# tkkim-robot/safe_control

Measured on AMD Instinct MI355X. Metric: QP solves/sec (batched agents), higher is better.
Workload: dtype f64; 1 GPU; 4096-agent batch DynamicUnicycle2D CBF-QP, 8 obstacles each (BASELINE configs[1]); agents_per_gpu=4096, obstacles=8, storage=f32, arithmetic=f64, launch=hipGraph

## Files before the change

safe_control_amd/csrc/cbf_qp_kernel.hpp:

```cpp
#pragma once
#include <hip/hip_runtime.h>

#include <type_traits>
#include <utility>

#include <cstdlib>

#include "sc_qp2.hpp"
#include "sc_group.hpp"

namespace sc {

#ifndef SC_COOP_MAX_AGENTS
#define SC_COOP_MAX_AGENTS 32768
#endif

static inline long long sc_coop_max_agents() {
    static const long long v = [] { const char* e = getenv("SC_COOP_MAX_AGENTS"); return e ? atoll(e) : (long long)SC_COOP_MAX_AGENTS; }();
    return v;
}
static inline bool sc_two_pass() {
    static const bool v = [] { const char* e = getenv("SC_CBFQP_TWO_PASS"); return !(e && e[0] == '0'); }();
    return v;
}
// ... 189 lines not shown
    const bool has_row = sub < K;
    const TIO* src = obs + (obs_shared ? 0 : (size_t)ag_i * K * 7) + (has_row ? sub * 7 : 0);
#pragma unroll
    for (int f = 0; f < 7; ++f) orow[f] = src[f];
    const V2 ur = reinterpret_cast<const V2*>(u_ref)[ag_i];
    const StateRow<TIO, MODEL> xs = load_state<TIO, MODEL>(X, ag_i);
    int nk = K;
    if (n_obs) nk = n_obs[ag_i];
    nk = nk < 0 ? 0 : (nk > K ? K : nk);
    fetch_arg_now(status_out); fetch_arg_now(h_out);
    fetch_arg_now(k.R); fetch_arg_now(k.g1); fetch_arg_now(k.g2);
    fetch_arg_now(k.lo0); fetch_arg_now(k.hi0); fetch_arg_now(k.lo1); fetch_arg_now(k.hi1); fetch_arg_now(k.hard);
#ifdef SC_EXP_LOADS
    if (active) {
        if (sub == 0) {
            V2 uo; uo.x = ur.x + xs.v[0] + xs.v[1]; uo.y = ur.y + xs.v[2] + xs.v[3];
            reinterpret_cast<V2*>(u_out)[agent] = uo;
            status_out[agent] = nk;
        }
        if (h_out && has_row) h_out[agent * K + sub] = orow[0] + orow[1] + orow[2] + orow[3] + orow[4] + orow[5] + orow[6];
    }
    return;
#endif
    const TC ur0 = TC(ur.x), ur1 = TC(ur.y);
    const Agent<TC> ag = to_agent<TIO, TC, MODEL>(xs);

    TC o[7];
#pragma unroll
    for (int f = 0; f < 7; ++f) o[f] = TC(orow[f]);
    TC h, a0, a1, cc;
#ifndef SC_EXP_NOROW
    const bool ok = cbf_row<TC, MODEL, false>(ag, o, k, a0, a1, cc, h);
#else
    const bool ok = true; a0 = o[0] - ag.x; a1 = o[1] - ag.y; cc = o[2]; h = o[3];
#endif
    const bool used = sub < nk;
    const bool bad_mine = used && !ok;
    a0 = used ? a0 : TC(0); a1 = used ? a1 : TC(0); cc = used ? cc : TC(0);
    if (active && h_out && has_row) h_out[agent * K + sub] = used ? TIO(h) : TIO(0);
    TC poison = TC(0);
    normalise_row(a0, a1, cc, poison);

    QpState<TC> S;
    qp_begin(S, ur0, ur1, k);
#ifndef SC_EXP_NOWALK
#ifndef SC_COOP_OLD_WALK
    if constexpr (G == 8) coop_solve_all8<TC>(S, K, sub, lane, a0, a1, cc, k);
    else if constexpr (G == 16) coop_solve_all16<TC>(S, K, sub, lane, a0, a1, cc, k);
    else
#endif
    coop_walk_violated<TC, G>(S, K, sub, lane, a0, a1, cc, k);
#endif
    qp_finish_box(S, k);
    TC worst = qp_row_margin(num<TC>::inf(), a0, a1, cc, S.u0, S.u1, poison);
    const bool nan_mine = !(poison == poison);
    worst = nan_mine ? -num<TC>::inf() : worst;
    if constexpr (G == 8) worst = min8_raw(worst);
    else if constexpr (G == 16) worst = min16_raw(worst);
    else worst = group_min<TC, G>(worst);
    const unsigned long long bad_mask = __builtin_amdgcn_ballot_w64(bad_mine);
    const bool bad_any = ((bad_mask >> (lane & ~(G - 1))) & (G == 64 ? ~0ull : ((1ull << G) - 1ull))) != 0ull;
    int st = qp_status(S, worst, TC(0), k);
    if (bad_any) st = SC_STATUS_BAD_OBSTACLE;
    TC u0 = S.u0, u1 = S.u1;
    if (st != SC_STATUS_OPTIMAL) { u0 = num<TC>::nan(); u1 = num<TC>::nan(); }
    if (active) {
        if (sub == 0) {
            V2 uo; uo.x = TIO(u0); uo.y = TIO(u1);
            reinterpret_cast<V2*>(u_out)[agent] = uo;
            status_out[agent] = st;
        }
    }
}

typedef double sc_d8 __attribute__((ext_vector_type(8)));
struct Coop8Consts {
    sc_d8 t0;
    sc_d8 t1;
    sc_d8 k0;
    sc_d8 k1;
    unsigned B;
};

__device__ __forceinline__ void normalise_row_as_generic(double& n0, double& n1, double& c, double& poison) {
    const double nn = __builtin_fma(n1, n1, n0 * n0);
    poison += 0.0 * (nn + c);
    double inv = rsqrt_(nn);
    if (__builtin_amdgcn_ballot_w64(!(nn > 0.0)) != 0ull) {
        asm volatile("");
        inv = nn > 0.0 ? inv : 1.0;
    }
    n0 *= inv; n1 *= inv; c *= inv;
}

template <typename T>
__device__ __forceinline__ T* at_byte(T* base, unsigned off) {
    using C = typename std::conditional<std::is_const<T>::value, const char, char>::type;
    return reinterpret_cast<T*>(reinterpret_cast<C*>(base) + off);
}

template <typename TIO, bool FULL, bool HAS_H, bool HARD>
__global__ __launch_bounds__(64) void cbfqp_coop8_du_kernel(const TIO* __restrict__ obs, const TIO* __restrict__ X,
                                                            const TIO* __restrict__ u_ref, TIO* __restrict__ u_out,
                                                            TIO* __restrict__ h_out, int* __restrict__ status_out,
                                                            const Coop8Consts c) {
#ifdef SC_EXP_EMPTY
    return;
#endif
    using TC = double;
    using V2 = typename vec2<TIO>::type;
    const unsigned lane = threadIdx.x;
    const unsigned sub = lane & 7u;
    const unsigned slot = blockIdx.x * 64u + lane;
    const unsigned agent = slot >> 3;
    bool active = true;
    if constexpr (!FULL) active = agent < c.B;
    const unsigned row_i = active ? slot : sub;
    const unsigned ag8 = row_i & ~7u;

    struct { TIO v[7]; } orow;
    __builtin_memcpy(&orow, at_byte(obs, __umul24(row_i, 7u * (unsigned)sizeof(TIO))), sizeof(orow));
    const V2 ur = *reinterpret_cast<const V2*>(at_byte(u_ref, ag8 * (unsigned)(sizeof(V2) / 8)));
    StateRow<TIO, SC_MODEL_DYNAMIC_UNICYCLE2D> xs;
    __builtin_memcpy(&xs, at_byte(X, ag8 * (unsigned)(sizeof(xs) / 8)), sizeof(xs));
    fetch_arg_now(c.t0); fetch_arg_now(c.t1); fetch_arg_now(c.k0); fetch_arg_now(c.k1);

    SinCosTab sc;
    sc.two_over_pi = c.t0[0]; sc.pio2_1 = c.t0[1]; sc.pio2_2 = c.t0[2]; sc.pio2_3 = c.t0[3];
    sc.s[0] = c.t0[4]; sc.s[1] = c.t0[5]; sc.s[2] = c.t0[6]; sc.s[3] = c.t0[7]; sc.s[4] = c.t1[0]; sc.s[5] = c.t1[1];
#pragma unroll
    for (int i = 0; i < 6; ++i) sc.c[i] = c.t1[2 + i];
    CbfConsts<TC> k;
    k.R = c.k0[0]; k.a1 = TC(0); k.a2 = TC(0); k.g1 = c.k0[1]; k.g2 = c.k0[2]; k.inv_dt = c.k0[3]; k.inv_dt2 = c.k0[4];
    k.lo0 = c.k0[5]; k.hi0 = c.k0[6]; k.lo1 = c.k0[7]; k.hi1 = c.k1[0]; k.inv_Lr = TC(0); k.inv_mass = TC(1); k.hard = HARD;
    BoxTol<TC> bt;
    bt.lo0 = c.k1[1]; bt.hi0 = c.k1[2]; bt.lo1 = c.k1[3]; bt.hi1 = c.k1[4];
    SolveLit<TC> lit;
    lit.tol_feas = c.k1[5]; lit.eps_par = c.k1[6]; lit.inf = c.k1[7];

    const TC ur0 = TC(ur.x), ur1 = TC(ur.y);
    Agent<TC> ag;
    ag.x = TC(xs.v[0]); ag.y = TC(xs.v[1]); ag.th = TC(xs.v[2]); ag.v = TC(xs.v[3]);
    sincos_tab_sfma(ag.th, sc, &ag.s, &ag.c);
    ag.f0 = ag.v * ag.c;
    ag.f1 = ag.v * ag.s;

    TC o[7];
#pragma unroll
    for (int f = 0; f < 7; ++f) o[f] = TC(orow.v[f]);
    TC h, a0, a1, cc;
    const bool ok = cbf_row<TC, SC_MODEL_DYNAMIC_UNICYCLE2D, false>(ag, o, k, a0, a1, cc, h);
    const bool bad_mine = !ok;
    if constexpr (HAS_H) {
        if (active) *at_byte(h_out, slot * (unsigned)sizeof(TIO)) = TIO(h);
    }
    TC poison = TC(0);
    normalise_row_as_generic(a0, a1, cc, poison);

    QpState<TC> S;
    qp_begin_raw(S, ur0, ur1, k);
    coop_solve_all8_full<TC>(S, (int)sub, (int)lane, a0, a1, cc, k, bt, lit);
    qp_finish_box_raw(S, k);
    TC worst = qp_row_margin_raw(a0, a1, cc, S.u0, S.u1, poison, lit);
    const bool nan_mine = !(poison == poison);
    worst = nan_mine ? -num<TC>::inf() : worst;
    worst = min8_raw(worst);
    int st = qp_status_lit(S, worst, TC(0), k, lit);
    if (__builtin_amdgcn_ballot_w64(bad_mine) != 0ull) {
        asm volatile("");
        const unsigned long long bad_mask = __builtin_amdgcn_ballot_w64(bad_mine);
        const bool bad_any = ((bad_mask >> (lane & ~7u)) & 0xffull) != 0ull;
        if (bad_any) st = SC_STATUS_BAD_OBSTACLE;
    }
    TC u0 = S.u0, u1 = S.u1;
    if (st != SC_STATUS_OPTIMAL) { u0 = num<TC>::nan(); u1 = num<TC>::nan(); }
    if (active && sub == 0) {
        V2 uo; uo.x = TIO(u0); uo.y = TIO(u1);
        reinterpret_cast<V2*>(u_out)[agent] = uo;
        status_out[agent] = st;
    }
}

#if defined(SC_EXP_GRID) && !defined(SC_EXP_EMPTY)
#error "SC_EXP_GRID needs SC_EXP_EMPTY: a kernel with a body would run past the batch"
#endif
static inline unsigned coop_grid(unsigned nblk) {
#ifdef SC_EXP_GRID
    return SC_EXP_GRID;
#else
    return nblk;
#endif
}

static inline bool sc_cbfqp_generic() {
    static const bool v = [] { const char* e = getenv("SC_CBFQP_GENERIC"); return e && e[0] == '1'; }();
    return v;
}

static inline double sc_quieted(double x) {
    if (x != x) {
        unsigned long long b;
        __builtin_memcpy(&b, &x, sizeof(b));
        b |= 0x0008000000000000ull;
        __builtin_memcpy(&x, &b, sizeof(b));
    }
    return x;
}

template <typename TIO>
static hipError_t launch_coop8_du(const sc_cbfqp_params& p, long long B, const void* X, const void* u_ref, const void* obs,
                                  void* u_out, int* status, void* h_out, hipStream_t stream) {
    const CbfConsts<double> k = make_consts<double>(p);
    const BoxTol<double> bt = box_tol(k);
    const SinCosTab t = make_sincos_tab();
    Coop8Consts c;
    c.t0 = sc_d8{t.two_over_pi, t.pio2_1, t.pio2_2, t.pio2_3, t.s[0], t.s[1], t.s[2], t.s[3]};
    c.t1 = sc_d8{t.s[4], t.s[5], t.c[0], t.c[1], t.c[2], t.c[3], t.c[4], t.c[5]};
    c.k0 = sc_d8{k.R, k.g1, k.g2, k.inv_dt, k.inv_dt2, sc_quieted(k.lo0), sc_quieted(k.hi0), sc_quieted(k.lo1)};
    c.k1 = sc_d8{sc_quieted(k.hi1), bt.lo0, bt.hi0, bt.lo1, bt.hi1, 1e-9, 1e-12, __builtin_huge_val()};
    c.B = (unsigned)B;
    const dim3 grid(coop_grid((unsigned)((B + 7) / 8))), block(64);
#define SC_GO(FULL, HAS_H, HARD)                                                                                             \
    hipLaunchKernelGGL((cbfqp_coop8_du_kernel<TIO, FULL, HAS_H, HARD>), grid, block, 0, stream, (const TIO*)obs, (const TIO*)X, \
                       (const TIO*)u_ref, (TIO*)u_out, (TIO*)h_out, status, c)
#define SC_GO_H(FULL, HAS_H) do { if (k.hard) SC_GO(FULL, HAS_H, true); else SC_GO(FULL, HAS_H, false); } while (0)
    if (B % 8 == 0) { if (h_out) SC_GO_H(true, true); else SC_GO_H(true, false); }
    else { if (h_out) SC_GO_H(false, true); else SC_GO_H(false, false); }
#undef SC_GO_H
#undef SC_GO
    return hipGetLastError();
}

template <typename TIO, typename TC, int G, int MODEL>
static hipError_t launch_coop(const sc_cbfqp_params& p, long long B, int K, const void* X, const void* u_ref,
                              const void* obs, const int* n_obs, void* u_out, int* status, void* h_out,
                              hipStream_t stream) {
    if constexpr (G == 8 && MODEL == SC_MODEL_DYNAMIC_UNICYCLE2D && sizeof(TC) == 8 && SC_COOP_WAVES == 1) {
        if (K == 8 && n_obs == nullptr && p.obs_shared == 0 && B >= 1 && B <= sc_coop_max_agents() &&
            B * 8 * 7 * (long long)sizeof(TIO) <= 0x7fffffffLL && B * 8 <= 0xffffffLL && !sc_cbfqp_generic())
            return launch_coop8_du<TIO>(p, B, X, u_ref, obs, u_out, status, h_out, stream);
    }
    constexpr int APW = 64 / G;
    const unsigned nblk = coop_grid((unsigned)((B + APW * SC_COOP_WAVES - 1) / (APW * SC_COOP_WAVES)));
    const CbfConsts<TC> k = make_consts<TC>(p);
    hipLaunchKernelGGL((cbfqp_coop_kernel<TIO, TC, G, MODEL>), dim3(nblk), dim3(64 * SC_COOP_WAVES), 0, stream,
                       (const TIO*)obs, (const TIO*)X, (const TIO*)u_ref, n_obs, B, K, (int)p.obs_shared,
                       (TIO*)u_out, status, (TIO*)h_out, k);
    return hipGetLastError();
}

template <typename TIO, typename TC, int KMAX, int MODEL>
__global__ __launch_bounds__(64) void cbfqp_kernel(const TIO* __restrict__ obs, const TIO* __restrict__ X,
                                                   const TIO* __restrict__ u_ref, const int* __restrict__ n_obs,
                                                   const long long B, const int K, const int obs_shared,
                                                   TIO* __restrict__ u_out, int* __restrict__ status_out,
                                                   TIO* __restrict__ h_out, const CbfConsts<TC> k) {
    extern __shared__ __attribute__((aligned(16))) unsigned char smem[];
    TIO* lobs = reinterpret_cast<TIO*>(smem);

    const int lane = threadIdx.x;
    const long long first = (long long)blockIdx.x * 64;
    const long long agent = first + lane;
    const int nag = (int)((B - first) < 64 ? (B - first) : 64);
    const bool active = lane < nag;
    const int row_elems = K * 7;

    if (obs_shared) {
        for (int e = lane; e < row_elems; e += 64) lobs[e] = obs[e];
    } else {
        const TIO* src = obs + (size_t)first * row_elems;
        const unsigned bytes = (unsigned)nag * row_elems * sizeof(TIO);
        if ((bytes & 15u) == 0 && ((reinterpret_cast<uintptr_t>(src) & 15u) == 0)) {
            wave_dma16(reinterpret_cast<const unsigned char*>(src), smem, bytes, lane);
        } else {
            const int total = nag * row_elems;
            for (int e = lane; e < total; e += 64) lobs[e] = src[e];
        }
    }

    using V2 = typename vec2<TIO>::type;
    const long long ag_i = active ? agent : 0;
    const V2 ur = reinterpret_cast<const V2*>(u_ref)[ag_i];
    const StateRow<TIO, MODEL> xs = load_state<TIO, MODEL>(X, ag_i);
    int nk = K;
    if (n_obs) nk = n_obs[ag_i];
    nk = !active ? K : (nk < 0 ? 0 : (nk > K ? K : nk));
    const TC ur0 = active ? TC(ur.x) : TC(0), ur1 = active ? TC(ur.y) : TC(0);
    const Agent<TC> ag = to_agent<TIO, TC, MODEL>(xs);

    asm volatile("s_waitcnt vmcnt(0)" ::: "memory");
    __syncthreads();

    const size_t stage_bytes = ((obs_shared ? (size_t)row_elems : (size_t)64 * row_elems) * sizeof(TIO) + 15) & ~(size_t)15;
    TC* rows = reinterpret_cast<TC*>(smem + stage_bytes);
    TIO* hl = reinterpret_cast<TIO*>(rows + (size_t)K * 3 * 64);
    const TIO* mine = lobs + (obs_shared ? 0 : lane * row_elems);
    int period = 32;
    while (((K * (32 / period)) & 31) != 0 && period > 1) period >>= 1;
    const int rot = obs_shared ? 0 : (lane / period) % K;
    bool bad_obs = false;
    TC poison = TC(0);
#pragma nounroll
// ... 152 lines not shown
```

safe_control_amd/csrc/sc_group.hpp:

```cpp
#pragma once
#include <hip/hip_runtime.h>

#include <utility>

#include "sc_qp2.hpp"

namespace sc {

template <int CTRL>
__device__ __forceinline__ float dpp_mov(float v) {
    return __int_as_float(__builtin_amdgcn_update_dpp(0, __float_as_int(v), CTRL, 0xf, 0xf, true));
}
template <int CTRL>
__device__ __forceinline__ double dpp_mov(double v) {
    const int lo = __builtin_amdgcn_update_dpp(0, __double2loint(v), CTRL, 0xf, 0xf, true);
    const int hi = __builtin_amdgcn_update_dpp(0, __double2hiint(v), CTRL, 0xf, 0xf, true);
    return __hiloint2double(hi, lo);
}
template <typename T, int G, int I>
__device__ __forceinline__ T group_bcast(T v, int sub) {
    if constexpr (G == 8) {
        const T q = dpp_mov<(I & 3) * 0x55>(v);
        const T m = dpp_mov<0x141>(q);
        return ((sub >> 2) == (I >> 2)) ? q : m;
// ... 93 lines not shown
__device__ __forceinline__ double keep_or_nan(bool keep, double v) {
    return __hiloint2double(keep ? __double2hiint(v) : 0x7ff80000, __double2loint(v));
}
template <typename T>
__device__ __forceinline__ T min8_raw(T v) {
    v = min_raw(v, dpp_mov<0xB1>(v)); v = min_raw(v, dpp_mov<0x4E>(v)); v = min_raw(v, dpp_mov<0x141>(v));
    return v;
}
template <typename T>
__device__ __forceinline__ T min16_raw(T v) { v = min8_raw(v); return min_raw(v, dpp_mov<0x140>(v)); }
template <int CTRL>
__device__ __forceinline__ int or_dpp(int v) { return v | __builtin_amdgcn_update_dpp(0, v, CTRL, 0xf, 0xf, true); }
template <int G>
__device__ __forceinline__ int group_or_bits(int v) {
    v = or_dpp<0xB1>(v); v = or_dpp<0x4E>(v); v = or_dpp<0x141>(v);
    if constexpr (G == 16) v = or_dpp<0x140>(v);
    return v;
}
template <int G>
__device__ __forceinline__ float group_pick(bool mine, float v) { return __int_as_float(group_or_bits<G>(mine ? __float_as_int(v) : 0)); }
template <int G>
__device__ __forceinline__ double group_pick(bool mine, double v) {
    const int lo = group_or_bits<G>(mine ? __double2loint(v) : 0), hi = group_or_bits<G>(mine ? __double2hiint(v) : 0);
    return __hiloint2double(hi, lo);
}

template <typename T>
__device__ __forceinline__ void clip_row_coop(LineQP<T>& L, bool& dead, T g0, T g1, T gc) {
    const T a = g0 * L.d0 + g1 * L.d1;
    const T r = g0 * L.p0 + (g1 * L.p1 + gc);
    const bool pos = a > num<T>::eps_par();
    const bool neg = !(a >= -num<T>::eps_par());
    const bool par_viol = r < -num<T>::tol_feas() * max_abs_one_raw(gc);
    const T q = r * rcp_(fabs_(a));
    dead |= !pos && !neg && par_viol;
    L.lo = max_neg_raw(L.lo, keep_or_nan(pos, q));
    L.hi = min_raw(L.hi, keep_or_nan(neg, q));
}

template <int G>
__device__ __forceinline__ bool group_first(unsigned long long m, int lane, int sub, bool& has) {
    const unsigned bits = (unsigned)(m >> (lane & ~(G - 1))) & ((1u << G) - 1u);
    has = bits != 0u;
    return sub == __builtin_ctz(bits | (1u << G));
}

template <typename TC, int... Xs>
__device__ __forceinline__ void clip_partners8(LineQP<TC>& L, bool& dead, TC a0, TC a1, TC cc, std::integer_sequence<int, Xs...>) {
    const TC m0 = dpp_mov<0x141>(a0), m1 = dpp_mov<0x141>(a1), mc = dpp_mov<0x141>(cc);
    (clip_row_coop(L, dead, group_xor8<TC, Xs + 1>(a0, m0), group_xor8<TC, Xs + 1>(a1, m1), group_xor8<TC, Xs + 1>(cc, mc)), ...);
}
template <typename TC, int G>
__device__ __forceinline__ void coop_pick_winner(QpState<TC>& S, const LineQP<TC>& L, bool ok, int sub, int lane) {
    const TC inf = num<TC>::inf();
    TC t = fmin_(fmax_(TC(0), L.lo), L.hi);
    const bool inverted = L.lo > L.hi;
    t = inverted ? TC(0.5) * (L.lo + L.hi) : t;
    const bool empty = L.lo > L.hi + num<TC>::tol_feas() * fmax_(TC(1), fmax_(fabs_(L.lo), fabs_(L.hi)));
    const TC v0 = L.p0 + t * L.d0, v1 = L.p1 + t * L.d1;
    const TC e0 = v0 - S.ur0, e1 = v1 - S.ur1;
    TC cost = e0 * e0 + e1 * e1;
    cost = (ok && !empty && (cost == cost)) ? cost : inf;
    TC best;
    if constexpr (G == 8) best = min8_raw(cost); else best = min16_raw(cost);
    bool has;
    const bool mine = group_first<G>(__builtin_amdgcn_ballot_w64((cost == best) && (best < inf)), lane, sub, has);
    const TC s0 = group_pick<G>(mine, v0), s1 = group_pick<G>(mine, v1);
    S.u0 = has ? s0 : S.u0;
    S.u1 = has ? s1 : S.u1;
}
template <typename TC>
__device__ __forceinline__ void coop_solve_all8(QpState<TC>& S, int K, int sub, int lane, TC a0, TC a1, TC cc,
                                                const CbfConsts<TC>& k) {
    const bool testable = (sub < K) && !((a0 == TC(0)) && (a1 == TC(0)));
    LineQP<TC> L;
    const bool viol = qp_row_violated(S, a0, a1, cc, L, k) && testable;
    if (__builtin_amdgcn_ballot_w64(viol) == 0ull) return;
    clip_box(L, k);
    bool dead = false;
    clip_partners8(L, dead, a0, a1, cc, std::make_integer_sequence<int, 7>{});
    coop_pick_winner<TC, 8>(S, L, viol && !dead, sub, lane);
}

template <typename T>
struct BoxTol { T lo0, hi0, lo1, hi1; };
template <typename T>
__host__ __device__ inline BoxTol<T> box_tol(const CbfConsts<T>& k) {
    const T tol = sizeof(T) == 8 ? T(1e-9) : T(1e-5f);
    BoxTol<T> b;
    b.lo0 = k.lo0 - tol; b.hi0 = k.hi0 + tol; b.lo1 = k.lo1 - tol; b.hi1 = k.hi1 + tol;
    return b;
}
template <typename T>
__device__ __forceinline__ void clip_box_tol(LineQP<T>& L, const CbfConsts<T>& k, const BoxTol<T>& bt) {
    const T inf = num<T>::inf();
    {
        const T r = rcp_(L.d0);
        const T t1 = (k.lo0 - L.p0) * r, t2 = (k.hi0 - L.p0) * r;
        const bool flat = L.d0 == T(0);
        const bool inside = (L.p0 >= bt.lo0) && (L.p0 <= bt.hi0);
        const T lo = flat ? (inside ? -inf : inf) : fmin_(t1, t2);
        const T hi = flat ? inf : fmax_(t1, t2);
        L.lo = lo; L.hi = hi;
    }
    {
        const T r = rcp_(L.d1);
        const T t1 = (k.lo1 - L.p1) * r, t2 = (k.hi1 - L.p1) * r;
        const bool flat = L.d1 == T(0);
        const bool inside = (L.p1 >= bt.lo1) && (L.p1 <= bt.hi1);
        const T lo = flat ? (inside ? -inf : inf) : fmin_(t1, t2);
        const T hi = flat ? inf : fmax_(t1, t2);
        L.lo = fmax_(L.lo, lo); L.hi = fmin_(L.hi, hi);
    }
}

__device__ __forceinline__ double max_raw_s(double a, double b) { double r; asm("v_max_f64 %0, %1, %2" : "=v"(r) : "v"(a), "s"(b)); return r; }
__device__ __forceinline__ double min_raw_s(double a, double b) { double r; asm("v_min_f64 %0, %1, %2" : "=v"(r) : "v"(a), "s"(b)); return r; }
__device__ __forceinline__ double max_zero_raw(double a) { double r; asm("v_max_f64 %0, %1, 0" : "=v"(r) : "v"(a)); return r; }
__device__ __forceinline__ double max_one_raw(double a) { double r; asm("v_max_f64 %0, %1, 1.0" : "=v"(r) : "v"(a)); return r; }
__device__ __forceinline__ double max_abs_abs_raw(double a, double b) { double r; asm("v_max_f64 %0, |%1|, |%2|" : "=v"(r) : "v"(a), "v"(b)); return r; }

__device__ __forceinline__ void qp_begin_raw(QpState<double>& S, double ur0, double ur1, const CbfConsts<double>& k) {
    S.ur0 = ur0; S.ur1 = ur1;
    S.u0 = min_raw_s(max_raw_s(ur0, k.lo0), k.hi0);
    S.u1 = min_raw_s(max_raw_s(ur1, k.lo1), k.hi1);
}
__device__ __forceinline__ void qp_finish_box_raw(QpState<double>& S, const CbfConsts<double>& k) {
    S.u0 = min_raw_s(max_raw_s(S.u0, k.lo0), k.hi0);
    S.u1 = min_raw_s(max_raw_s(S.u1, k.lo1), k.hi1);
}
template <typename T>
struct SolveLit { T tol_feas, eps_par, inf; };

__device__ __forceinline__ double qp_row_margin_raw(double a0, double a1, double ci, double u0, double u1, double& poison,
                                                    const SolveLit<double>& lit) {
    const double s = a0 * u0 + (a1 * u1 + ci);
    const double m = s + lit.tol_feas * max_abs_one_raw(ci);
    poison += 0.0 * s;
    return fmin_(lit.inf, m);
}
__device__ __forceinline__ int qp_status_lit(const QpState<double>& S, double worst, double poison, const CbfConsts<double>& k,
                                             const SolveLit<double>& lit) {
    const bool finite = (poison == poison) && (fabs_(S.ur0 + S.ur1) < lit.inf);
    const bool box_ok = (k.lo0 <= k.hi0) && (k.lo1 <= k.hi1);
    return (!(worst >= 0.0) || !finite || !box_ok) ? SC_STATUS_INFEASIBLE : SC_STATUS_OPTIMAL;
}

template <typename T>
__device__ __forceinline__ void clip_box_tol_lazy(LineQP<T>& L, const CbfConsts<T>& k, const BoxTol<T>& bt) {
    const T r0 = rcp_(L.d0), r1 = rcp_(L.d1);
    const T t1 = (k.lo0 - L.p0) * r0, t2 = (k.hi0 - L.p0) * r0;
    const T t3 = (k.lo1 - L.p1) * r1, t4 = (k.hi1 - L.p1) * r1;
    const bool flat = (L.d0 == T(0)) || (L.d1 == T(0));
    L.lo = fmax_(fmin_(t1, t2), fmin_(t3, t4));
    L.hi = fmin_(fmax_(t1, t2), fmax_(t3, t4));
    if (__builtin_amdgcn_ballot_w64(flat) != 0ull) clip_box_tol(L, k, bt);
}

__device__ __forceinline__ double min_abs_abs_raw(double a, double b) { double r; asm("v_min_f64 %0, |%1|, |%2|" : "=v"(r) : "v"(a), "v"(b)); return r; }
__device__ __forceinline__ double min_abs_raw(double a, double b) { double r; asm("v_min_f64 %0, %1, |%2|" : "=v"(r) : "v"(a), "v"(b)); return r; }
__device__ __forceinline__ double clip_row_coop_lazy(LineQP<double>& L, double eps, double g0, double g1, double gc) {
    const double a = g0 * L.d0 + g1 * L.d1;
    const double r = g0 * L.p0 + (g1 * L.p1 + gc);
    const bool pos = a > eps;
    const bool neg = !(a >= -eps);
    const double q = r * rcp_(fabs_(a));
    L.lo = max_neg_raw(L.lo, keep_or_nan(pos, q));
    L.hi = min_raw(L.hi, keep_or_nan(neg, q));
    return a;
}
template <int X>
__device__ __forceinline__ double clip_partner8_lazy(LineQP<double>& L, double eps, double a0, double a1, double cc, double m0, double m1,
                                                     double mc) {
    return clip_row_coop_lazy(L, eps, group_xor8<double, X>(a0, m0), group_xor8<double, X>(a1, m1), group_xor8<double, X>(cc, mc));
}
__device__ __forceinline__ double clip_partners8_lazy(LineQP<double>& L, double eps, double a0, double a1, double cc) {
    const double m0 = dpp_mov<0x141>(a0), m1 = dpp_mov<0x141>(a1), mc = dpp_mov<0x141>(cc);
    const double x1 = clip_partner8_lazy<1>(L, eps, a0, a1, cc, m0, m1, mc);
    const double x2 = clip_partner8_lazy<2>(L, eps, a0, a1, cc, m0, m1, mc);
    double amin = min_abs_abs_raw(x1, x2);
    amin = min_abs_raw(amin, clip_partner8_lazy<3>(L, eps, a0, a1, cc, m0, m1, mc));
    amin = min_abs_raw(amin, clip_partner8_lazy<4>(L, eps, a0, a1, cc, m0, m1, mc));
    amin = min_abs_raw(amin, clip_partner8_lazy<5>(L, eps, a0, a1, cc, m0, m1, mc));
    amin = min_abs_raw(amin, clip_partner8_lazy<6>(L, eps, a0, a1, cc, m0, m1, mc));
    amin = min_abs_raw(amin, clip_partner8_lazy<7>(L, eps, a0, a1, cc, m0, m1, mc));
    return amin;
}
template <typename T>
__device__ __forceinline__ bool row_dead_coop(const LineQP<T>& L, T g0, T g1, T gc) {
    const T a = g0 * L.d0 + g1 * L.d1;
    const T r = g0 * L.p0 + (g1 * L.p1 + gc);
    const bool pos = a > num<T>::eps_par();
    const bool neg = !(a >= -num<T>::eps_par());
    const bool par_viol = r < -num<T>::tol_feas() * max_abs_one_raw(gc);
    return !pos && !neg && par_viol;
}
template <typename TC>
__device__ __forceinline__ bool partners8_dead(const LineQP<TC>& L, TC a0, TC a1, TC cc) {
    bool dead = false;
#pragma nounroll
    for (int x = 1; x < 8; ++x) dead |= row_dead_coop(L, __shfl_xor(a0, x, 8), __shfl_xor(a1, x, 8), __shfl_xor(cc, x, 8));
    return dead;
}

__device__ __forceinline__ void coop_pick_winner8_raw(QpState<double>& S, const LineQP<double>& L, bool ok, int sub, int lane,
                                                      const SolveLit<double>& lit) {
    using TC = double;
    const TC inf = num<TC>::inf();
    TC t = min_raw(max_zero_raw(L.lo), L.hi);
    const bool inverted = L.lo > L.hi;
    t = inverted ? TC(0.5) * (L.lo + L.hi) : t;
    const bool empty = L.lo > L.hi + lit.tol_feas * max_one_raw(max_abs_abs_raw(L.lo, L.hi));
    const TC v0 = L.p0 + t * L.d0, v1 = L.p1 + t * L.d1;
    const TC e0 = v0 - S.ur0, e1 = v1 - S.ur1;
    TC cost = e0 * e0 + e1 * e1;
    cost = (ok && !empty && (cost == cost)) ? cost : inf;
    const TC best = min8_raw(cost);
    bool has;
    const bool mine = group_first<8>(__builtin_amdgcn_ballot_w64((cost == best) && (best < lit.inf)), lane, sub, has);
    const TC s0 = group_pick<8>(mine, v0), s1 = group_pick<8>(mine, v1);
    S.u0 = has ? s0 : S.u0;
    S.u1 = has ? s1 : S.u1;
}

template <typename TC>
__device__ __forceinline__ void coop_solve_all8_full(QpState<TC>& S, int sub, int lane, TC a0, TC a1, TC cc,
                                                     const CbfConsts<TC>& k, const BoxTol<TC>& bt, const SolveLit<TC>& lit) {
    const bool testable = !((a0 == TC(0)) && (a1 == TC(0)));
    LineQP<TC> L;
    const bool viol = qp_row_violated(S, a0, a1, cc, L, k) && testable;
    if (__builtin_amdgcn_ballot_w64(viol) == 0ull) return;
    clip_box_tol_lazy(L, k, bt);
    const TC amin = clip_partners8_lazy(L, lit.eps_par, a0, a1, cc);
    bool dead = false;
    if (__builtin_amdgcn_ballot_w64(amin <= lit.eps_par) != 0ull)
        dead = partners8_dead(L, a0, a1, cc);
    coop_pick_winner8_raw(S, L, viol && !dead, sub, lane, lit);
}

template <typename TC, int... Rs>
__device__ __forceinline__ void clip_partners16(LineQP<TC>& L, bool& dead, TC a0, TC a1, TC cc, std::integer_sequence<int, Rs...>) {
    (clip_row_coop(L, dead, dpp_mov<0x121 + Rs>(a0), dpp_mov<0x121 + Rs>(a1), dpp_mov<0x121 + Rs>(cc)), ...);
}
template <typename TC>
__device__ __forceinline__ void coop_solve_all16(QpState<TC>& S, int K, int sub, int lane, TC a0, TC a1, TC cc,
                                                 const CbfConsts<TC>& k) {
    const bool testable = (sub < K) && !((a0 == TC(0)) && (a1 == TC(0)));
    LineQP<TC> L;
    const bool viol = qp_row_violated(S, a0, a1, cc, L, k) && testable;
    if (__builtin_amdgcn_ballot_w64(viol) == 0ull) return;
    clip_box(L, k);
    bool dead = false;
    clip_partners16(L, dead, a0, a1, cc, std::make_integer_sequence<int, 15>{});
    coop_pick_winner<TC, 16>(S, L, viol && !dead, sub, lane);
}

}
```

safe_control_amd/csrc/sc_math.hpp:

```cpp
#pragma once
#include <hip/hip_runtime.h>
#include <cmath>
#include <cstdint>

namespace sc {

template <typename T> struct num;
template <> struct num<float> {
    static __device__ __forceinline__ float inf() { return __builtin_huge_valf(); }
    static __device__ __forceinline__ float nan() { return __builtin_nanf(""); }
    static __device__ __forceinline__ float eps_par() { return 1e-5f; }
    static __device__ __forceinline__ float tol_feas() { return 1e-5f; }
};
template <> struct num<double> {
    static __device__ __forceinline__ double inf() { return __builtin_huge_val(); }
    static __device__ __forceinline__ double nan() { return __builtin_nan(""); }
    static __device__ __forceinline__ double eps_par() { return 1e-12; }
    static __device__ __forceinline__ double tol_feas() { return 1e-9; }
};

__device__ __forceinline__ void sincos_(float x, float* s, float* c) { sincosf(x, s, c); }
__device__ __forceinline__ void sincos_(double x, double* s, double* c) {
    if (!(fabs(x) < 1.0e5)) { sincos(x, s, c); return; }
    const double k = rint(x * 0.63661977236758138);
    double r = __builtin_fma(-k, 1.5707963267948966, x);
    r = __builtin_fma(-k, 6.123233995736766e-17, r);
    r = __builtin_fma(-k, -1.4973849048591698e-33, r);
    const double z = r * r;
    double ps = __builtin_fma(z, 1.58969099521155010221e-10, -2.50507602534068634195e-08);
    ps = __builtin_fma(z, ps, 2.75573137070700676789e-06);
    ps = __builtin_fma(z, ps, -1.98412698298579493134e-04);
    ps = __builtin_fma(z, ps, 8.33333333332248946124e-03);
    const double ks = __builtin_fma(z * r, __builtin_fma(z, ps, -1.66666666666666324348e-01), r);
    double pc = __builtin_fma(z, -1.13596475577881948265e-11, 2.08757232129817482790e-09);
    pc = __builtin_fma(z, pc, -2.75573143513906633035e-07);
    pc = __builtin_fma(z, pc, 2.48015872894767294178e-05);
    pc = __builtin_fma(z, pc, -1.38888888888741095749e-03);
    pc = __builtin_fma(z, pc, 4.16666666666666019037e-02);
    const double hz = 0.5 * z, w = 1.0 - hz;
    const double kc = w + (((1.0 - w) - hz) + z * (z * pc));
    const int n = (int)k & 3;
    const double sv = (n & 1) ? kc : ks, cv = (n & 1) ? ks : kc;
    *s = (n & 2) ? -sv : sv;
    *c = ((n + 1) & 2) ? -cv : cv;
}
struct SinCosTab {
    double two_over_pi, pio2_1, pio2_2, pio2_3;
    double s[6];
    double c[6];
};
__host__ __device__ inline SinCosTab make_sincos_tab() {
    SinCosTab t;
    t.two_over_pi = 0.63661977236758138;
    t.pio2_1 = 1.5707963267948966; t.pio2_2 = 6.123233995736766e-17; t.pio2_3 = -1.4973849048591698e-33;
    t.s[0] = 1.58969099521155010221e-10; t.s[1] = -2.50507602534068634195e-08; t.s[2] = 2.75573137070700676789e-06;
    t.s[3] = -1.98412698298579493134e-04; t.s[4] = 8.33333333332248946124e-03; t.s[5] = -1.66666666666666324348e-01;
    t.c[0] = -1.13596475577881948265e-11; t.c[1] = 2.08757232129817482790e-09; t.c[2] = -2.75573143513906633035e-07;
    t.c[3] = 2.48015872894767294178e-05; t.c[4] = -1.38888888888741095749e-03; t.c[5] = 4.16666666666666019037e-02;
    return t;
}
__device__ __forceinline__ void sincos_tab(double x, const SinCosTab& t, double* s, double* c) {
    if (!(fabs(x) < 1.0e5)) { sincos(x, s, c); return; }
    const double k = rint(x * t.two_over_pi);
    double r = __builtin_fma(-k, t.pio2_1, x);
    r = __builtin_fma(-k, t.pio2_2, r);
    r = __builtin_fma(-k, t.pio2_3, r);
    const double z = r * r;
    double ps = __builtin_fma(z, t.s[0], t.s[1]);
    ps = __builtin_fma(z, ps, t.s[2]);
    ps = __builtin_fma(z, ps, t.s[3]);
    ps = __builtin_fma(z, ps, t.s[4]);
    const double ks = __builtin_fma(z * r, __builtin_fma(z, ps, t.s[5]), r);
    double pc = __builtin_fma(z, t.c[0], t.c[1]);
    pc = __builtin_fma(z, pc, t.c[2]);
    pc = __builtin_fma(z, pc, t.c[3]);
    pc = __builtin_fma(z, pc, t.c[4]);
    pc = __builtin_fma(z, pc, t.c[5]);
    const double hz = 0.5 * z, w = 1.0 - hz;
    const double kc = w + (((1.0 - w) - hz) + z * (z * pc));
    const int n = (int)k & 3;
    const double sv = (n & 1) ? kc : ks, cv = (n & 1) ? ks : kc;
    *s = (n & 2) ? -sv : sv;
    *c = ((n + 1) & 2) ? -cv : cv;
}
__device__ __forceinline__ double fma_sconst(double a, double b, double c) {
    double d;
    asm("v_fma_f64 %0, %1, %2, %3" : "=v"(d) : "v"(a), "v"(b), "s"(c));
    return d;
}
__device__ __forceinline__ void sincos_tab_sfma(double x, const SinCosTab& t, double* s, double* c) {
    if (!(fabs(x) < 1.0e5)) { sincos(x, s, c); return; }
    const double k = rint(x * t.two_over_pi);
    double r = __builtin_fma(-k, t.pio2_1, x);
    r = __builtin_fma(-k, t.pio2_2, r);
    r = __builtin_fma(-k, t.pio2_3, r);
    const double z = r * r;
    double ps = __builtin_fma(z, t.s[0], t.s[1]);
    ps = fma_sconst(z, ps, t.s[2]);
    ps = fma_sconst(z, ps, t.s[3]);
    ps = fma_sconst(z, ps, t.s[4]);
    const double ks = __builtin_fma(z * r, fma_sconst(z, ps, t.s[5]), r);
    double pc = __builtin_fma(z, t.c[0], t.c[1]);
    pc = fma_sconst(z, pc, t.c[2]);
    pc = fma_sconst(z, pc, t.c[3]);
    pc = fma_sconst(z, pc, t.c[4]);
    pc = fma_sconst(z, pc, t.c[5]);
    const double hz = 0.5 * z, w = 1.0 - hz;
    const double kc = w + (((1.0 - w) - hz) + z * (z * pc));
    const int n = (int)k & 3;
    const double sv = (n & 1) ? kc : ks, cv = (n & 1) ? ks : kc;
    *s = (n & 2) ? -sv : sv;
    *c = ((n + 1) & 2) ? -cv : cv;
}
__device__ __forceinline__ float sqrt_(float x) { return sqrtf(x); }
__device__ __forceinline__ double sqrt_(double x) { return sqrt(x); }
__device__ __forceinline__ float fabs_(float x) { return fabsf(x); }
__device__ __forceinline__ double fabs_(double x) { return fabs(x); }
__device__ __forceinline__ float fmax_(float a, float b) { return fmaxf(a, b); }
__device__ __forceinline__ double fmax_(double a, double b) { return fmax(a, b); }
__device__ __forceinline__ float fmin_(float a, float b) { return fminf(a, b); }
__device__ __forceinline__ double fmin_(double a, double b) { return fmin(a, b); }
__device__ __forceinline__ float pow_(float a, float b) { return powf(a, b); }
__device__ __forceinline__ double pow_(double a, double b) { return pow(a, b); }
__device__ __forceinline__ float rint_(float a) { return rintf(a); }
__device__ __forceinline__ double rint_(double a) { return rint(a); }
__device__ __forceinline__ float atan2_(float a, float b) { return atan2f(a, b); }
__device__ __forceinline__ double atan2_(double a, double b) { return atan2(a, b); }
__device__ __forceinline__ float floor_(float a) { return floorf(a); }
__device__ __forceinline__ double floor_(double a) { return floor(a); }
__device__ __forceinline__ bool finite_(float a) { return __builtin_isfinite(a); }
__device__ __forceinline__ bool finite_(double a) { return __builtin_isfinite(a); }

template <typename T>
__device__ __forceinline__ T powi_chain(T x, int n) {
    T r = T(1), b = x;
    while (n) {
        if (n & 1) r *= b;
        b *= b;
        n >>= 1;
    }
    return r;
}

__device__ __forceinline__ float fmod_(float a, float b) { return fmodf(a, b); }
__device__ __forceinline__ double fmod_(double a, double b) { return fmod(a, b); }

template <typename T>
__device__ __forceinline__ T pymod(T x, T m) {
    T r = fmod_(x, m);
    if (r < T(0)) r += m;
    return r;
}

template <typename T>
__device__ __forceinline__ T angle_normalize(T x) {
    const T pi = T(3.14159265358979323846);
    return pymod(x + pi, T(2) * pi) - pi;
}

}
```

Measured before the change: 1.682 billion solves/s.

## Split coop8 kernel into fast path with wave-level fallback to generic solver

```diff
diff --git a/safe_control_amd/csrc/cbf_qp_kernel.hpp b/safe_control_amd/csrc/cbf_qp_kernel.hpp
--- a/safe_control_amd/csrc/cbf_qp_kernel.hpp
+++ b/safe_control_amd/csrc/cbf_qp_kernel.hpp
@@ -295,21 +295,74 @@
     unsigned B;
 };
 
-__device__ __forceinline__ void normalise_row_as_generic(double& n0, double& n1, double& c, double& poison) {
+template <bool HARD>
+__device__ __forceinline__ void circle_row_du_as_generic(const Agent<double>& a, const double* o, const CbfConsts<double>& k,
+                                                         double neg_beta, double& n0, double& n1, double& c, double& h) {
+    const double ex = a.x - o[0], ey = a.y - o[1];
+    const double dmin = o[2] + k.R;
+    h = __builtin_fma(dmin, dmin * neg_beta, __builtin_fma(ex, ex, ey * ey));
+    const double hdot = 2.0 * __builtin_fma(ex, a.f0, ey * a.f1);
+    const double dhd0 = 2.0 * a.f0, dhd1 = 2.0 * a.f1;
+    n1 = 2.0 * __builtin_fma(ey, a.f0, -(ex * a.f1));
+    n0 = 2.0 * __builtin_fma(ex, a.c, ey * a.s);
+    const double Lf = __builtin_fma(dhd0, a.f0, dhd1 * a.f1);
+    if constexpr (HARD) c = __builtin_fma(h, k.inv_dt2, (2.0 * hdot) * k.inv_dt) + Lf;
+    else c = __builtin_fma(k.g2, h, __builtin_fma(k.g1, hdot, Lf));
+}
+
+__device__ __forceinline__ bool normalise_row_fast(double& n0, double& n1, double& c, double& poison) {
     const double nn = __builtin_fma(n1, n1, n0 * n0);
     poison += 0.0 * (nn + c);
-    double inv = rsqrt_(nn);
-    if (__builtin_amdgcn_ballot_w64(!(nn > 0.0)) != 0ull) {
-        asm volatile("");
-        inv = nn > 0.0 ? inv : 1.0;
-    }
+    const double inv = rsqrt_(nn);
     n0 *= inv; n1 *= inv; c *= inv;
+    return !(nn > 0.0);
 }
 
 template <typename T>
 __device__ __forceinline__ T* at_byte(T* base, unsigned off) {
     using C = typename std::conditional<std::is_const<T>::value, const char, char>::type;
     return reinterpret_cast<T*>(reinterpret_cast<C*>(base) + off);
+}
+
+template <typename TIO, bool HAS_H>
+__device__ __forceinline__ void coop8_generic_body(const TIO* orow, typename vec2<TIO>::type ur,
+                                                   const StateRow<TIO, SC_MODEL_DYNAMIC_UNICYCLE2D>& xs, bool active,
+                                                   unsigned slot, int sub, int lane, const CbfConsts<double>& k,
+                                                   TIO* __restrict__ h_out, typename vec2<TIO>::type& uo, int& st) {
+    using TC = double;
+    constexpr int MODEL = SC_MODEL_DYNAMIC_UNICYCLE2D;
+    int K = 8, nk = 8;
+    asm volatile("" : "+s"(K), "+s"(nk));
+    const TC ur0 = TC(ur.x), ur1 = TC(ur.y);
+    const Agent<TC> ag = to_agent<TIO, TC, MODEL>(xs);
+    TC o[7];
+#pragma unroll
+    for (int f = 0; f < 7; ++f) o[f] = TC(orow[f]);
+    TC h, a0, a1, cc;
+    const bool ok = cbf_row<TC, MODEL, false>(ag, o, k, a0, a1, cc, h);
+    const bool used = sub < nk;
+    const bool bad_mine = used && !ok;
+    a0 = used ? a0 : TC(0); a1 = used ? a1 : TC(0); cc = used ? cc : TC(0);
+    if constexpr (HAS_H) {
+        if (active && sub < K) *at_byte(h_out, slot * (unsigned)sizeof(TIO)) = used ? TIO(h) : TIO(0);
+    }
+    TC poison = TC(0);
+    normalise_row(a0, a1, cc, poison);
+    QpState<TC> S;
+    qp_begin(S, ur0, ur1, k);
+    coop_solve_all8<TC>(S, K, sub, lane, a0, a1, cc, k);
+    qp_finish_box(S, k);
+    TC worst = qp_row_margin(num<TC>::inf(), a0, a1, cc, S.u0, S.u1, poison);
+    const bool nan_mine = !(poison == poison);
+    worst = nan_mine ? -num<TC>::inf() : worst;
+    worst = min8_raw(worst);
+    const unsigned long long bad_mask = __builtin_amdgcn_ballot_w64(bad_mine);
+    const bool bad_any = ((bad_mask >> (lane & ~7)) & 0xffull) != 0ull;
+    st = qp_status(S, worst, TC(0), k);
+    if (bad_any) st = SC_STATUS_BAD_OBSTACLE;
+    TC u0 = S.u0, u1 = S.u1;
+    if (st != SC_STATUS_OPTIMAL) { u0 = num<TC>::nan(); u1 = num<TC>::nan(); }
+    uo.x = TIO(u0); uo.y = TIO(u1);
 }
 
 template <typename TIO, bool FULL, bool HAS_H, bool HARD>
@@ -338,61 +391,66 @@
     __builtin_memcpy(&xs, at_byte(X, ag8 * (unsigned)(sizeof(xs) / 8)), sizeof(xs));
     fetch_arg_now(c.t0); fetch_arg_now(c.t1); fetch_arg_now(c.k0); fetch_arg_now(c.k1);
 
+    CbfConsts<TC> k;
+    k.R = c.k0[0]; k.a1 = TC(0); k.a2 = TC(0); k.g1 = c.k0[1]; k.g2 = c.k0[2]; k.inv_dt = c.k0[3]; k.inv_dt2 = c.k0[4];
+    k.lo0 = c.k0[5]; k.hi0 = c.k0[6]; k.lo1 = c.k0[7]; k.hi1 = c.k1[0]; k.inv_Lr = TC(0); k.inv_mass = TC(1); k.hard = HARD;
+    SolveLit<TC> lit;
+    lit.th_max = c.k1[1]; lit.neg_beta = c.k1[2]; lit.tol_feas = c.k1[5]; lit.eps_par = c.k1[6]; lit.inf = c.k1[7];
+
+    const TC th = TC(xs.v[2]);
+    const bool early = (orow.v[6] != TIO(0)) || !(fabs(th) < lit.th_max);
+    const auto store_u_status = [&](V2 uo, int st) {
+        if (active && sub == 0) {
+            reinterpret_cast<V2*>(u_out)[agent] = uo;
+            status_out[agent] = st;
+        }
+    };
+    if (__builtin_expect(__builtin_amdgcn_ballot_w64(early) != 0ull, 0)) {
+        V2 uo; int st;
+        coop8_generic_body<TIO, HAS_H>(orow.v, ur, xs, active, slot, (int)sub, (int)lane, k, h_out, uo, st);
+        store_u_status(uo, st);
+        return;
+    }
     SinCosTab sc;
     sc.two_over_pi = c.t0[0]; sc.pio2_1 = c.t0[1]; sc.pio2_2 = c.t0[2]; sc.pio2_3 = c.t0[3];
     sc.s[0] = c.t0[4]; sc.s[1] = c.t0[5]; sc.s[2] = c.t0[6]; sc.s[3] = c.t0[7]; sc.s[4] = c.t1[0]; sc.s[5] = c.t1[1];
 #pragma unroll
     for (int i = 0; i < 6; ++i) sc.c[i] = c.t1[2 + i];
-    CbfConsts<TC> k;
-    k.R = c.k0[0]; k.a1 = TC(0); k.a2 = TC(0); k.g1 = c.k0[1]; k.g2 = c.k0[2]; k.inv_dt = c.k0[3]; k.inv_dt2 = c.k0[4];
-    k.lo0 = c.k0[5]; k.hi0 = c.k0[6]; k.lo1 = c.k0[7]; k.hi1 = c.k1[0]; k.inv_Lr = TC(0); k.inv_mass = TC(1); k.hard = HARD;
-    BoxTol<TC> bt;
-    bt.lo0 = c.k1[1]; bt.hi0 = c.k1[2]; bt.lo1 = c.k1[3]; bt.hi1 = c.k1[4];
-    SolveLit<TC> lit;
-    lit.tol_feas = c.k1[5]; lit.eps_par = c.k1[6]; lit.inf = c.k1[7];
-
     const TC ur0 = TC(ur.x), ur1 = TC(ur.y);
     Agent<TC> ag;
-    ag.x = TC(xs.v[0]); ag.y = TC(xs.v[1]); ag.th = TC(xs.v[2]); ag.v = TC(xs.v[3]);
+    ag.x = TC(xs.v[0]); ag.y = TC(xs.v[1]); ag.th = th; ag.v = TC(xs.v[3]);
     sincos_tab_sfma(ag.th, sc, &ag.s, &ag.c);
     ag.f0 = ag.v * ag.c;
     ag.f1 = ag.v * ag.s;
 
-    TC o[7];
-#pragma unroll
-    for (int f = 0; f < 7; ++f) o[f] = TC(orow.v[f]);
+    TC o[3];
+#pragma unroll
+    for (int f = 0; f < 3; ++f) o[f] = TC(orow.v[f]);
     TC h, a0, a1, cc;
-    const bool ok = cbf_row<TC, SC_MODEL_DYNAMIC_UNICYCLE2D, false>(ag, o, k, a0, a1, cc, h);
-    const bool bad_mine = !ok;
+    circle_row_du_as_generic<HARD>(ag, o, k, lit.neg_beta, a0, a1, cc, h);
     if constexpr (HAS_H) {
         if (active) *at_byte(h_out, slot * (unsigned)sizeof(TIO)) = TIO(h);
     }
     TC poison = TC(0);
-    normalise_row_as_generic(a0, a1, cc, poison);
+    const unsigned long long odd_row = __builtin_amdgcn_ballot_w64(normalise_row_fast(a0, a1, cc, poison));
 
     QpState<TC> S;
     qp_begin_raw(S, ur0, ur1, k);
-    coop_solve_all8_full<TC>(S, (int)sub, (int)lane, a0, a1, cc, k, bt, lit);
+    const unsigned long long odd_solve = coop_solve_all8_fast<TC>(S, (int)sub, (int)lane, a0, a1, cc, k, lit);
     qp_finish_box_raw(S, k);
     TC worst = qp_row_margin_raw(a0, a1, cc, S.u0, S.u1, poison, lit);
     const bool nan_mine = !(poison == poison);
     worst = nan_mine ? -num<TC>::inf() : worst;
     worst = min8_raw(worst);
     int st = qp_status_lit(S, worst, TC(0), k, lit);
-    if (__builtin_amdgcn_ballot_w64(bad_mine) != 0ull) {
-        asm volatile("");
-        const unsigned long long bad_mask = __builtin_amdgcn_ballot_w64(bad_mine);
-        const bool bad_any = ((bad_mask >> (lane & ~7u)) & 0xffull) != 0ull;
-        if (bad_any) st = SC_STATUS_BAD_OBSTACLE;
-    }
     TC u0 = S.u0, u1 = S.u1;
     if (st != SC_STATUS_OPTIMAL) { u0 = num<TC>::nan(); u1 = num<TC>::nan(); }
-    if (active && sub == 0) {
-        V2 uo; uo.x = TIO(u0); uo.y = TIO(u1);
-        reinterpret_cast<V2*>(u_out)[agent] = uo;
-        status_out[agent] = st;
-    }
-}
+    V2 uo; uo.x = TIO(u0); uo.y = TIO(u1);
+    if (__builtin_expect((odd_row | odd_solve) != 0ull, 0))
+        coop8_generic_body<TIO, HAS_H>(orow.v, ur, xs, active, slot, (int)sub, (int)lane, k, h_out, uo, st);
+    store_u_status(uo, st);
+}
+
 
 #if defined(SC_EXP_GRID) && !defined(SC_EXP_EMPTY)
 #error "SC_EXP_GRID needs SC_EXP_EMPTY: a kernel with a body would run past the batch"
@@ -424,13 +482,12 @@
 static hipError_t launch_coop8_du(const sc_cbfqp_params& p, long long B, const void* X, const void* u_ref, const void* obs,
                                   void* u_out, int* status, void* h_out, hipStream_t stream) {
     const CbfConsts<double> k = make_consts<double>(p);
-    const BoxTol<double> bt = box_tol(k);
     const SinCosTab t = make_sincos_tab();
     Coop8Consts c;
     c.t0 = sc_d8{t.two_over_pi, t.pio2_1, t.pio2_2, t.pio2_3, t.s[0], t.s[1], t.s[2], t.s[3]};
     c.t1 = sc_d8{t.s[4], t.s[5], t.c[0], t.c[1], t.c[2], t.c[3], t.c[4], t.c[5]};
     c.k0 = sc_d8{k.R, k.g1, k.g2, k.inv_dt, k.inv_dt2, sc_quieted(k.lo0), sc_quieted(k.hi0), sc_quieted(k.lo1)};
-    c.k1 = sc_d8{sc_quieted(k.hi1), bt.lo0, bt.hi0, bt.lo1, bt.hi1, 1e-9, 1e-12, __builtin_huge_val()};
+    c.k1 = sc_d8{sc_quieted(k.hi1), 1.0e5, -1.01, 0.0, 0.0, 1e-9, 1e-12, __builtin_huge_val()};
     c.B = (unsigned)B;
     const dim3 grid(coop_grid((unsigned)((B + 7) / 8))), block(64);
 #define SC_GO(FULL, HAS_H, HARD)                                                                                             \
diff --git a/safe_control_amd/csrc/sc_group.hpp b/safe_control_amd/csrc/sc_group.hpp
--- a/safe_control_amd/csrc/sc_group.hpp
+++ b/safe_control_amd/csrc/sc_group.hpp
@@ -199,37 +199,6 @@
     coop_pick_winner<TC, 8>(S, L, viol && !dead, sub, lane);
 }
 
-template <typename T>
-struct BoxTol { T lo0, hi0, lo1, hi1; };
-template <typename T>
-__host__ __device__ inline BoxTol<T> box_tol(const CbfConsts<T>& k) {
-    const T tol = sizeof(T) == 8 ? T(1e-9) : T(1e-5f);
-    BoxTol<T> b;
-    b.lo0 = k.lo0 - tol; b.hi0 = k.hi0 + tol; b.lo1 = k.lo1 - tol; b.hi1 = k.hi1 + tol;
-    return b;
-}
-template <typename T>
-__device__ __forceinline__ void clip_box_tol(LineQP<T>& L, const CbfConsts<T>& k, const BoxTol<T>& bt) {
-    const T inf = num<T>::inf();
-    {
-        const T r = rcp_(L.d0);
-        const T t1 = (k.lo0 - L.p0) * r, t2 = (k.hi0 - L.p0) * r;
-        const bool flat = L.d0 == T(0);
-        const bool inside = (L.p0 >= bt.lo0) && (L.p0 <= bt.hi0);
-        const T lo = flat ? (inside ? -inf : inf) : fmin_(t1, t2);
-        const T hi = flat ? inf : fmax_(t1, t2);
-        L.lo = lo; L.hi = hi;
-    }
-    {
-        const T r = rcp_(L.d1);
-        const T t1 = (k.lo1 - L.p1) * r, t2 = (k.hi1 - L.p1) * r;
-        const bool flat = L.d1 == T(0);
-        const bool inside = (L.p1 >= bt.lo1) && (L.p1 <= bt.hi1);
-        const T lo = flat ? (inside ? -inf : inf) : fmin_(t1, t2);
-        const T hi = flat ? inf : fmax_(t1, t2);
-        L.lo = fmax_(L.lo, lo); L.hi = fmin_(L.hi, hi);
-    }
-}
 
 __device__ __forceinline__ double max_raw_s(double a, double b) { double r; asm("v_max_f64 %0, %1, %2" : "=v"(r) : "v"(a), "s"(b)); return r; }
 __device__ __forceinline__ double min_raw_s(double a, double b) { double r; asm("v_min_f64 %0, %1, %2" : "=v"(r) : "v"(a), "s"(b)); return r; }
@@ -247,7 +216,7 @@
     S.u1 = min_raw_s(max_raw_s(S.u1, k.lo1), k.hi1);
 }
 template <typename T>
-struct SolveLit { T tol_feas, eps_par, inf; };
+struct SolveLit { T tol_feas, eps_par, inf, th_max, neg_beta; };
 
 __device__ __forceinline__ double qp_row_margin_raw(double a0, double a1, double ci, double u0, double u1, double& poison,
                                                     const SolveLit<double>& lit) {
@@ -264,14 +233,12 @@
 }
 
 template <typename T>
-__device__ __forceinline__ void clip_box_tol_lazy(LineQP<T>& L, const CbfConsts<T>& k, const BoxTol<T>& bt) {
+__device__ __forceinline__ void clip_box_fast(LineQP<T>& L, const CbfConsts<T>& k) {
     const T r0 = rcp_(L.d0), r1 = rcp_(L.d1);
     const T t1 = (k.lo0 - L.p0) * r0, t2 = (k.hi0 - L.p0) * r0;
     const T t3 = (k.lo1 - L.p1) * r1, t4 = (k.hi1 - L.p1) * r1;
-    const bool flat = (L.d0 == T(0)) || (L.d1 == T(0));
     L.lo = fmax_(fmin_(t1, t2), fmin_(t3, t4));
     L.hi = fmin_(fmax_(t1, t2), fmax_(t3, t4));
-    if (__builtin_amdgcn_ballot_w64(flat) != 0ull) clip_box_tol(L, k, bt);
 }
 
 __device__ __forceinline__ double min_abs_abs_raw(double a, double b) { double r; asm("v_min_f64 %0, |%1|, |%2|" : "=v"(r) : "v"(a), "v"(b)); return r; }
@@ -303,23 +270,6 @@
     amin = min_abs_raw(amin, clip_partner8_lazy<7>(L, eps, a0, a1, cc, m0, m1, mc));
     return amin;
 }
-template <typename T>
-__device__ __forceinline__ bool row_dead_coop(const LineQP<T>& L, T g0, T g1, T gc) {
-    const T a = g0 * L.d0 + g1 * L.d1;
-    const T r = g0 * L.p0 + (g1 * L.p1 + gc);
-    const bool pos = a > num<T>::eps_par();
-    const bool neg = !(a >= -num<T>::eps_par());
-    const bool par_viol = r < -num<T>::tol_feas() * max_abs_one_raw(gc);
-    return !pos && !neg && par_viol;
-}
-template <typename TC>
-__device__ __forceinline__ bool partners8_dead(const LineQP<TC>& L, TC a0, TC a1, TC cc) {
-    bool dead = false;
-#pragma nounroll
-    for (int x = 1; x < 8; ++x) dead |= row_dead_coop(L, __shfl_xor(a0, x, 8), __shfl_xor(a1, x, 8), __shfl_xor(cc, x, 8));
-    return dead;
-}
-
 __device__ __forceinline__ void coop_pick_winner8_raw(QpState<double>& S, const LineQP<double>& L, bool ok, int sub, int lane,
                                                       const SolveLit<double>& lit) {
     using TC = double;
@@ -341,18 +291,16 @@
 }
 
 template <typename TC>
-__device__ __forceinline__ void coop_solve_all8_full(QpState<TC>& S, int sub, int lane, TC a0, TC a1, TC cc,
-                                                     const CbfConsts<TC>& k, const BoxTol<TC>& bt, const SolveLit<TC>& lit) {
+__device__ __forceinline__ unsigned long long coop_solve_all8_fast(QpState<TC>& S, int sub, int lane, TC a0, TC a1, TC cc,
+                                                     const CbfConsts<TC>& k, const SolveLit<TC>& lit) {
     const bool testable = !((a0 == TC(0)) && (a1 == TC(0)));
     LineQP<TC> L;
     const bool viol = qp_row_violated(S, a0, a1, cc, L, k) && testable;
-    if (__builtin_amdgcn_ballot_w64(viol) == 0ull) return;
-    clip_box_tol_lazy(L, k, bt);
+    if (__builtin_amdgcn_ballot_w64(viol) == 0ull) return 0ull;
+    clip_box_fast(L, k);
     const TC amin = clip_partners8_lazy(L, lit.eps_par, a0, a1, cc);
-    bool dead = false;
-    if (__builtin_amdgcn_ballot_w64(amin <= lit.eps_par) != 0ull)
-        dead = partners8_dead(L, a0, a1, cc);
-    coop_pick_winner8_raw(S, L, viol && !dead, sub, lane, lit);
+    coop_pick_winner8_raw(S, L, viol, sub, lane, lit);
+    return __builtin_amdgcn_ballot_w64((L.d0 == TC(0)) || (L.d1 == TC(0)) || (amin <= lit.eps_par));
 }
 
 template <typename TC, int... Rs>
diff --git a/safe_control_amd/csrc/sc_math.hpp b/safe_control_amd/csrc/sc_math.hpp
--- a/safe_control_amd/csrc/sc_math.hpp
+++ b/safe_control_amd/csrc/sc_math.hpp
@@ -89,7 +89,6 @@
     return d;
 }
 __device__ __forceinline__ void sincos_tab_sfma(double x, const SinCosTab& t, double* s, double* c) {
-    if (!(fabs(x) < 1.0e5)) { sincos(x, s, c); return; }
     const double k = rint(x * t.two_over_pi);
     double r = __builtin_fma(-k, t.pio2_1, x);
     r = __builtin_fma(-k, t.pio2_2, r);
```

After: 1.784 billion solves/s (median of 6 runs). 1.06x the previous value.
